# gattia/pyfocusr

Measured on AMD Instinct MI355X. Metric: lowest-k eigenpairs/sec + KNN-correspondence wall-clock, 250k-vertex mesh pair k=5, higher is better.
Workload: dtype f64

## Files before the change

### include/pyfocusr_hip.h

```cpp
#ifndef PYFOCUSR_HIP_H
#define PYFOCUSR_HIP_H

#include <stddef.h>
#include <stdint.h>

#ifdef __cplusplus
extern "C" {
#endif

#define PF_VERSION 1

#define PF_OK 0
#define PF_E_ARG (-1)
#define PF_E_HIP (-2)
#define PF_E_DEGENERATE (-3)
#define PF_E_STATE (-4)
#define PF_E_PERSIST_TIMEOUT (-5)

#define PF_OP_RW 0
#define PF_OP_SYM 1

typedef struct pf_ctx pf_ctx;
typedef struct pf_graph pf_graph;
typedef struct pf_mesh pf_mesh;
// ... 67 lines not shown
int pf_persist_enable(int on);
int pf_persist_two_step(int level);
int pf_persist_pair_halves(int on);
int pf_persist_clock(pf_ctx* ctx, double* kernel_ms, int64_t* launches, int reset);
typedef struct pf_persist_info {
    int32_t enabled;
    int32_t two_step;
    int32_t owner;
    int32_t timeouts;
    int64_t launches;
    int64_t launches_two_step;
    int32_t suspended_for;
    int32_t rearms;
    int32_t owner_switches;
    int32_t hold_ticks;
} pf_persist_info;
int pf_persist_state(pf_ctx* ctx , pf_persist_info* out);
int pf_persist_test_hook(int n_launches);
int pf_cheb(pf_graph* g, int32_t op, int32_t src, int32_t dst, int32_t degree, double c, double e, double rho);
int pf_cheb2(pf_graph* ga, int32_t op_a, int32_t src_a, int32_t dst_a, int32_t degree_a, double c_a, double e_a, double rho_a,
             pf_graph* gb, int32_t op_b, int32_t src_b, int32_t dst_b, int32_t degree_b, double c_b, double e_b, double rho_b);
int pf_dots(pf_graph* g, int32_t w, int32_t first, int32_t count, double* out);
int pf_orth(pf_graph* g, int32_t w, int32_t first, int32_t count, double* h, double* nrm);
int pf_orth_begin(pf_graph* g, int32_t w, int32_t first, int32_t count, int32_t normalize);
int pf_orth_end(pf_graph* g, double* h, double* nrm);
int pf_orth_begin2(pf_graph* ga, int32_t w_a, int32_t first_a, int32_t count_a, int32_t normalize_a, pf_graph* gb, int32_t w_b,
                   int32_t first_b, int32_t count_b, int32_t normalize_b);
int pf_orth_cheb2(pf_graph* ga, pf_graph* gb, const int32_t* orth, const int32_t* cheb_i, const double* cheb_d);
int pf_orth_redone(pf_graph* g);
int pf_orth_strict(pf_graph* g, int32_t on);
int pf_orth_device_passes(pf_graph* g, int32_t on);
int pf_orth_split(pf_graph* g, int32_t first2, int32_t split);
int pf_orth_one_launch(int32_t on);
int pf_scale(pf_graph* g, int32_t slot, double alpha);
int pf_combine(pf_graph* g, int32_t src_first, int32_t m, const double* Y, int32_t k, int32_t dst_first);
int pf_resnorm(pf_graph* g, int32_t ax, int32_t x, double lam, double* out);
int pf_gram(pf_graph* g, int32_t first_a, int32_t count_a, int32_t first_b, int32_t count_b, double* out);
int pf_resnorms(pf_graph* g, int32_t ax_first, int32_t x_first, const double* lam, int32_t count, double* out);
int pf_finalize_vectors(pf_graph* g, int32_t first, int32_t count, int32_t from_sym, int32_t minmax,
                        double* out);
int pf_finalize_vectors_begin(pf_graph* g, int32_t first, int32_t count, int32_t from_sym, int32_t minmax, double* out);
int pf_finalize_vectors_end(pf_graph* g);
int pf_final_remap_begin(pf_graph* g, const int32_t* col, const double* sign, int32_t count, double* out);
int pf_host_alloc(size_t bytes, void** out);
int pf_host_free(void* p);
int pf_host_detach(void* p);
int pf_final_rows(pf_graph* g, const int64_t* rows, int64_t n_rows, double* out);
int pf_point_rows(pf_graph* g, const int64_t* rows, int64_t n_rows, double* out);
int pf_spmv_host(pf_graph* g, int32_t op, const double* x, double* y);
int pf_mean_filter(pf_graph* g, const double* values, int32_t ncols, int32_t iterations, double* out);

int pf_knn1(pf_ctx* ctx, const double* ref, int64_t n_ref, const double* qry, int64_t n_qry, int32_t d,
            int64_t* idx_out, double* d2_out);
int pf_knn_mode(pf_ctx* ctx, int32_t mode);
int pf_knn_tree_stats(pf_ctx* ctx, int32_t enable_counting, int64_t* leaves_scanned, int64_t* supers_opened);
int pf_knn_count(pf_ctx* ctx, int32_t enable_counting, int64_t* pairs);
int pf_knn_wave_stats(pf_ctx* ctx, double* sum_us, double* max_us, int64_t* waves, int64_t* max_candidates, double* detail);
int pf_knn(pf_ctx* ctx, const double* ref, int64_t n_ref, const double* qry, int64_t n_qry, int32_t d, int32_t k,
           int64_t* idx_out, double* d2_out);
int pf_knn_topk(pf_ctx* ctx, const double* ref, int64_t n_ref, const double* qry, int64_t n_qry, int32_t d, int32_t k,
                int64_t* idx_out, double* d2_out);
int pf_knn1_graphs(pf_graph* ref_g, pf_graph* qry_g, int32_t d, const int32_t* col_ref, const double* scale_ref,
                   const int32_t* col_qry, const double* scale_qry, int64_t* idx_out, double* d2_out);
int pf_knn1_blocks(pf_ctx* ctx, const double* ref_block, int64_t n_ref, int32_t ref_stride, const double* qry_block,
                   int64_t n_qry, int32_t qry_stride, int32_t d, const int32_t* col_ref, const double* scale_ref,
                   const int32_t* col_qry, const double* scale_qry, int64_t* idx_out, double* d2_out);
// ... 132 lines not shown
```

### pyfocusr_amd/_hip.py

```python
import atexit
import ctypes as C
import os
import threading
import weakref

import numpy as np

_HERE = os.path.dirname(os.path.abspath(__file__))
LIB_PATH = os.environ.get("PYFOCUSR_HIP_LIB", os.path.join(_HERE, "csrc", "libpyfocusr_hip.so"))

PF_OP_RW = 0
PF_OP_SYM = 1

_f64p = C.POINTER(C.c_double)
_i32p = C.POINTER(C.c_int32)
_i64p = C.POINTER(C.c_int64)


class HipUnavailable(RuntimeError):
    pass


class PfError(RuntimeError):
    def __init__(self, code, msg):
# ... 51 lines not shown
    "pf_graph_build_cotan": (C.c_int, [C.c_void_p, C.c_int32, C.POINTER(C.c_void_p)]),
    "pf_graph_cotan_info": (C.c_int, [C.c_void_p, C.POINTER(C.c_double), C.POINTER(C.c_double)]),
    "pf_graph_cotan_download": (C.c_int, [C.c_void_p, _f64p, _f64p, _f64p]),
    "pf_cotan_apply": (C.c_int, [C.c_void_p, _f64p, C.c_int32, _f64p]),
    "pf_graph_free": (None, [C.c_void_p]),
    "pf_graph_get_info": (C.c_int, [C.c_void_p, C.POINTER(GraphInfo)]),
    "pf_graph_download": (C.c_int, [C.c_void_p, _i32p, _i32p, _f64p, _f64p, _f64p, _f64p, _i32p]),
    "pf_ws_ensure": (C.c_int, [C.c_void_p, C.c_int32]),
    "pf_ws_upload": (C.c_int, [C.c_void_p, C.c_int32, _f64p]),
    "pf_ws_download": (C.c_int, [C.c_void_p, C.c_int32, C.c_int32, _f64p]),
    "pf_ws_copy": (C.c_int, [C.c_void_p, C.c_int32, C.c_int32, C.c_int32]),
    "pf_start_vector": (C.c_int, [C.c_void_p, C.c_int32, C.c_uint64]),
    "pf_mask_isolated": (C.c_int, [C.c_void_p, C.c_int32]),
    "pf_lock_null_vectors": (C.c_int, [C.c_void_p, C.c_int32, _i32p]),
    "pf_spmv": (C.c_int, [C.c_void_p, C.c_int32, C.c_int32, C.c_int32]),
    "pf_spmv_multi": (C.c_int, [C.c_void_p, C.c_int32, C.c_int32, C.c_int32, C.c_int32]),
    "pf_knn_mode": (C.c_int, [C.c_void_p, C.c_int32]),
    "pf_knn_tree_stats": (C.c_int, [C.c_void_p, C.c_int32, C.POINTER(C.c_int64), C.POINTER(C.c_int64)]),
    "pf_persist_enable": (C.c_int, [C.c_int]),
    "pf_persist_two_step": (C.c_int, [C.c_int]),
    "pf_persist_pair_halves": (C.c_int, [C.c_int]),
    "pf_persist_clock": (C.c_int, [C.c_void_p, C.POINTER(C.c_double), C.POINTER(C.c_int64), C.c_int]),
    "pf_persist_state": (C.c_int, [C.c_void_p, C.c_void_p]),
    "pf_persist_test_hook": (C.c_int, [C.c_int]),
    "pf_cheb": (C.c_int, [C.c_void_p, C.c_int32, C.c_int32, C.c_int32, C.c_int32, C.c_double, C.c_double, C.c_double]),
    "pf_cheb2": (C.c_int, [C.c_void_p, C.c_int32, C.c_int32, C.c_int32, C.c_int32, C.c_double, C.c_double, C.c_double,
                           C.c_void_p, C.c_int32, C.c_int32, C.c_int32, C.c_int32, C.c_double, C.c_double, C.c_double]),
    "pf_dots": (C.c_int, [C.c_void_p, C.c_int32, C.c_int32, C.c_int32, _f64p]),
    "pf_orth": (C.c_int, [C.c_void_p, C.c_int32, C.c_int32, C.c_int32, _f64p, _f64p]),
    "pf_orth_begin": (C.c_int, [C.c_void_p, C.c_int32, C.c_int32, C.c_int32, C.c_int32]),
    "pf_orth_end": (C.c_int, [C.c_void_p, _f64p, _f64p]),
    "pf_orth_split": (C.c_int, [C.c_void_p, C.c_int32, C.c_int32]),
    "pf_orth_one_launch": (C.c_int, [C.c_int32]),
    "pf_orth_begin2": (C.c_int, [C.c_void_p, C.c_int32, C.c_int32, C.c_int32, C.c_int32, C.c_void_p, C.c_int32, C.c_int32, C.c_int32,
                                 C.c_int32]),
    "pf_orth_cheb2": (C.c_int, [C.c_void_p, C.c_void_p, _i32p, _i32p, _f64p]),
    "pf_eigsort_costs": (C.c_int, [C.c_void_p, C.c_void_p, _i64p, C.c_int64, _i64p, C.c_int64, C.c_int32, _i32p, _f64p, _i32p, _f64p, _f64p,
                                   _i64p]),
    "pf_orth_redone": (C.c_int, [C.c_void_p]),
    "pf_orth_strict": (C.c_int, [C.c_void_p, C.c_int32]),
    "pf_scale": (C.c_int, [C.c_void_p, C.c_int32, C.c_double]),
    "pf_combine": (C.c_int, [C.c_void_p, C.c_int32, C.c_int32, _f64p, C.c_int32, C.c_int32]),
    "pf_resnorm": (C.c_int, [C.c_void_p, C.c_int32, C.c_int32, C.c_double, _f64p]),
    "pf_gram": (C.c_int, [C.c_void_p, C.c_int32, C.c_int32, C.c_int32, C.c_int32, _f64p]),
    "pf_resnorms": (C.c_int, [C.c_void_p, C.c_int32, C.c_int32, _f64p, C.c_int32, _f64p]),
    "pf_finalize_vectors": (C.c_int, [C.c_void_p, C.c_int32, C.c_int32, C.c_int32, C.c_int32, _f64p]),
    "pf_finalize_vectors_begin": (C.c_int, [C.c_void_p, C.c_int32, C.c_int32, C.c_int32, C.c_int32, _f64p]),
    "pf_finalize_vectors_end": (C.c_int, [C.c_void_p]),
    "pf_final_remap_begin": (C.c_int, [C.c_void_p, _i32p, _f64p, C.c_int32, _f64p]),
    "pf_host_alloc": (C.c_int, [C.c_size_t, C.POINTER(C.c_void_p)]),
    "pf_host_free": (C.c_int, [C.c_void_p]),
    "pf_final_rows": (C.c_int, [C.c_void_p, _i64p, C.c_int64, _f64p]),
    "pf_point_rows": (C.c_int, [C.c_void_p, _i64p, C.c_int64, _f64p]),
    "pf_spmv_host": (C.c_int, [C.c_void_p, C.c_int32, _f64p, _f64p]),
    "pf_mean_filter": (C.c_int, [C.c_void_p, _f64p, C.c_int32, C.c_int32, _f64p]),
    "pf_knn1": (C.c_int, [C.c_void_p, _f64p, C.c_int64, _f64p, C.c_int64, C.c_int32, _i64p, _f64p]),
    "pf_knn": (C.c_int, [C.c_void_p, _f64p, C.c_int64, _f64p, C.c_int64, C.c_int32, C.c_int32, _i64p, _f64p]),
    "pf_knn_topk": (C.c_int, [C.c_void_p, _f64p, C.c_int64, _f64p, C.c_int64, C.c_int32, C.c_int32, _i64p, _f64p]),
    "pf_knn1_graphs": (C.c_int, [C.c_void_p, C.c_void_p, C.c_int32, _i32p, _f64p, _i32p, _f64p, _i64p, _f64p]),
    "pf_knn1_blocks": (C.c_int, [C.c_void_p, C.c_void_p, C.c_int64, C.c_int32, C.c_void_p, C.c_int64, C.c_int32, C.c_int32,
                                 _i32p, _f64p, _i32p, _f64p, _i64p, _f64p]),
    "pf_final_device": (C.c_int, [C.c_void_p, C.POINTER(C.c_void_p), _i64p, _i32p]),
    "pf_knn_upload": (C.c_int, [C.c_void_p, _f64p, C.c_int64, _f64p, C.c_int64, C.c_int32]),
    "pf_knn_run": (C.c_int, [C.c_void_p]),
    "pf_knn_download": (C.c_int, [C.c_void_p, _i64p, _f64p]),
    "pf_eigs_smallest": (C.c_int, [C.c_void_p, C.c_int32, C.c_int32, _f64p, _f64p, C.POINTER(C.c_int32), C.POINTER(EigsStats)]),
# ... 154 lines not shown
    for ptr in blocks:
        _lib.pf_host_free(C.c_void_p(ptr))


def pinned_empty(shape, dtype=np.float64):
    lib = load_library()
    dtype = np.dtype(dtype)
    count = int(np.prod(shape)) if len(shape) else 1
    nbytes = max(count * dtype.itemsize, 1)
    nbytes = (nbytes + 4095) & ~4095
    ptr = None
    with _pinned_lock:
        free = _pinned_free.get(nbytes)
        if free:
            ptr = free.pop()
            _pinned_cached[0] -= nbytes
    if ptr is None:
        p = C.c_void_p()
        _check(lib.pf_host_alloc(C.c_size_t(nbytes), C.byref(p)))
        ptr = int(p.value)
    buf = (C.c_char * nbytes).from_address(ptr)
    buf._pf_block = _PinnedBlock(ptr, nbytes)
    return np.frombuffer(buf, dtype=dtype, count=count).reshape(shape)


def persist_enable(on=True):
    _check(load_library().pf_persist_enable(int(bool(on))))


def orth_one_launch(on=True):
    _check(load_library().pf_orth_one_launch(int(bool(on))))


def persist_two_step(level=1):
    _check(load_library().pf_persist_two_step(int(level)))


def persist_pair_halves(on=True):
    _check(load_library().pf_persist_pair_halves(int(bool(on))))


def persist_clock(ctx, reset=False):
    ms, n = C.c_double(0.0), C.c_int64(0)
    _check(load_library().pf_persist_clock(ctx._h, C.byref(ms), C.byref(n), int(bool(reset))))
    return ms.value, n.value


class _PersistInfo(C.Structure):
    _fields_ = [("enabled", C.c_int32), ("two_step", C.c_int32), ("owner", C.c_int32), ("timeouts", C.c_int32),
                ("launches", C.c_int64), ("launches_two_step", C.c_int64), ("suspended_for", C.c_int32), ("rearms", C.c_int32),
                ("owner_switches", C.c_int32), ("hold_ticks", C.c_int32)]


def persist_state(ctx=None):
    info = _PersistInfo()
    _check(load_library().pf_persist_state(None if ctx is None else ctx._h, C.byref(info)))
    return {name: int(getattr(info, name)) for name, _ in _PersistInfo._fields_}


def persist_test_hook(n_launches=1):
    _check(load_library().pf_persist_test_hook(int(n_launches)))


def _check(code):
    if code != 0:
        raise PfError(code, load_library().pf_last_error().decode("utf-8", "replace"))
# ... 1035 lines not shown
```

### pyfocusr_amd/csrc/pf_eigsort.hip

```cpp
#include <float.h>
#include <string.h>

#include <vector>

#include "pf_internal.h"

extern "C" int pf_knn1_blocks(pf_ctx* c, const double* ref_block, int64_t n_ref, int32_t ref_stride, const double* qry_block, int64_t n_qry,
                              int32_t qry_stride, int32_t d, const int32_t* col_ref, const double* scale_ref, const int32_t* col_qry,
                              const double* scale_qry, int64_t* idx_out, double* d2_out);

namespace {

constexpr int ES_SORT_THREADS = 1024;
constexpr int ES_MAX_SAMPLES = 16384;
constexpr int ES_RED_THREADS = 256;

__global__ __launch_bounds__(PF_BLOCK) void k_es_gather(const double* __restrict__ fin, int32_t fc, const double* __restrict__ pts,
                                                        const int64_t* __restrict__ rows, int64_t m, int32_t k,
                                                        const int32_t* __restrict__ col, const double* __restrict__ sign,
                                                        double* __restrict__ vals, double* __restrict__ raw) {
    const int64_t e = (int64_t)blockIdx.x * PF_BLOCK + threadIdx.x;
    if (e >= m * (k + 3)) return;
    const int64_t c = e / m, r = e - c * m;
    if (c < k) vals[c * m + r] = fin[rows[r] * fc + col[c]] * sign[c];
// ... 3 lines not shown
__global__ __launch_bounds__(ES_RED_THREADS) void k_es_minmax(const double* __restrict__ raw, int64_t m, double* __restrict__ lohi) {
    __shared__ double slo[ES_RED_THREADS], shi[ES_RED_THREADS];
    const int c = blockIdx.x;
    double lo = INFINITY, hi = -INFINITY;
    for (int64_t r = threadIdx.x; r < m; r += ES_RED_THREADS) {
        const double v = raw[r * 3 + c];
        lo = v < lo ? v : lo;
        hi = v > hi ? v : hi;
    }
    slo[threadIdx.x] = lo;
    shi[threadIdx.x] = hi;
    __syncthreads();
    for (int s = ES_RED_THREADS / 2; s > 0; s >>= 1) {
        if (threadIdx.x < s) {
            slo[threadIdx.x] = slo[threadIdx.x + s] < slo[threadIdx.x] ? slo[threadIdx.x + s] : slo[threadIdx.x];
            shi[threadIdx.x] = shi[threadIdx.x + s] > shi[threadIdx.x] ? shi[threadIdx.x + s] : shi[threadIdx.x];
        }
        __syncthreads();
    }
    if (threadIdx.x == 0) {
        lohi[c] = slo[0];
        lohi[3 + c] = shi[0];
    }
}

__global__ __launch_bounds__(PF_BLOCK) void k_es_normalize(const double* __restrict__ raw, const double* __restrict__ lohi, int64_t m,
                                                           double* __restrict__ out) {
    const int64_t e = (int64_t)blockIdx.x * PF_BLOCK + threadIdx.x;
    if (e >= m * 3) return;
    const int c = (int)(e % 3);
    out[e] = (raw[e] - lohi[c]) / (lohi[3 + c] - lohi[c]);
}

__global__ __launch_bounds__(ES_SORT_THREADS) void k_es_sort_log(const double* __restrict__ vals_t, const double* __restrict__ vals_s,
                                                                 int64_t mt, int64_t ms, int32_t k, double* __restrict__ lt,
                                                                 double* __restrict__ ls, double* __restrict__ lsf) {
    extern __shared__ double buf[];
    const int b = blockIdx.x;
    const int64_t m = b < k ? mt : ms;
    int n_pow2 = 2;
    while (n_pow2 < m) n_pow2 <<= 1;
    const double* src = b < k ? vals_t + (int64_t)b * m : vals_s + (int64_t)(b - k) * m;
    for (int i = threadIdx.x; i < n_pow2; i += ES_SORT_THREADS) buf[i] = i < m ? src[i] : INFINITY;
    __syncthreads();
    for (int size = 2; size <= n_pow2; size <<= 1) {
        for (int stride = size >> 1; stride > 0; stride >>= 1) {
            for (int t = threadIdx.x; t < n_pow2 / 2; t += ES_SORT_THREADS) {
                const int pos = 2 * t - (t & (stride - 1));
                const double a = buf[pos], c = buf[pos + stride];
                const bool up = (pos & size) == 0;
                if ((a > c) == up) {
                    buf[pos] = c;
                    buf[pos + stride] = a;
                }
            }
            __syncthreads();
        }
    }
    const double eps = DBL_EPSILON;
    if (b < k) {
        for (int64_t i = threadIdx.x; i < m; i += ES_SORT_THREADS) lt[(int64_t)b * m + i] = log(buf[i] + 0.5 + eps);
    } else {
        const int64_t o = (int64_t)(b - k) * m;
        for (int64_t i = threadIdx.x; i < m; i += ES_SORT_THREADS) {
            ls[o + i] = log(buf[i] + 0.5 + eps);
            lsf[o + i] = log(-buf[m - 1 - i] + 0.5 + eps);
        }
    }
}

__device__ __forceinline__ double es_block_sum(double v, double* sh) {
    sh[threadIdx.x] = v;
    __syncthreads();
    for (int s = ES_RED_THREADS / 2; s > 0; s >>= 1) {
        if (threadIdx.x < s) sh[threadIdx.x] += sh[threadIdx.x + s];
        __syncthreads();
    }
    const double r = sh[0];
    __syncthreads();
    return r;
}

__global__ __launch_bounds__(ES_RED_THREADS) void k_es_w1(const double* __restrict__ lt, const double* __restrict__ ls,
                                                          const double* __restrict__ lsf, int64_t mt, int64_t ms, int32_t k,
                                                          double* __restrict__ out) {
    __shared__ double sh[ES_RED_THREADS];
    const int i = blockIdx.x / k, j = blockIdx.x - i * k;
    const double unit = 1.0 / ((double)mt * (double)ms);
    double acc = 0.0, accf = 0.0;
    for (int64_t a = threadIdx.x; a < mt; a += ES_RED_THREADS) {
        const double t = lt[(int64_t)i * mt + a];
        const int64_t lo = a * ms, hi = lo + ms;
        for (int64_t b = lo / mt; b < ms && b * mt < hi; ++b) {
            const int64_t from = b * mt > lo ? b * mt : lo, to = (b + 1) * mt < hi ? (b + 1) * mt : hi;
            const double len = (double)(to - from) * unit;
            acc += len * fabs(t - ls[(int64_t)j * ms + b]);
            accf += len * fabs(t - lsf[(int64_t)j * ms + b]);
        }
    }
    acc = es_block_sum(acc, sh);
    accf = es_block_sum(accf, sh);
// ... 14 lines not shown
        const double t = vals_t[(int64_t)i * m + r], s = (nn >= 0 && nn < ms) ? vals_s[(int64_t)j * ms + nn] : NAN;
        const double d0 = s - t, d1 = -s - t;
        a += d0 * d0;
        f += d1 * d1;
    }
    a = es_block_sum(a, sh);
    f = es_block_sum(f, sh);
    if (threadIdx.x == 0) {
        out[2 * k * k + i * k + j] = sqrt(a) / (double)m;
        out[3 * k * k + i * k + j] = sqrt(f) / (double)m;
    }
}

}

extern "C" int pf_eigsort_costs(pf_graph* gt, pf_graph* gs, const int64_t* rows_t, int64_t mt, const int64_t* rows_s, int64_t ms, int32_t k,
                                const int32_t* col_t, const double* sign_t, const int32_t* col_s, const double* sign_s, double* out,
                                int64_t* idx_out) {
    PF_CHECK(gt && gs && rows_t && rows_s && col_t && sign_t && col_s && sign_s && out && idx_out, PF_E_ARG,
             "pf_eigsort_costs: NULL argument");
    PF_CHECK(gt->ctx == gs->ctx, PF_E_ARG, "pf_eigsort_costs: the two graphs must share one ctx");
    PF_CHECK(mt >= 1 && mt <= ES_MAX_SAMPLES && ms >= 1 && ms <= ES_MAX_SAMPLES && k >= 1 && k <= 16, PF_E_ARG,
             "pf_eigsort_costs: %lld / %lld samples (1..%d), k = %d (1..16)", (long long)mt, (long long)ms, ES_MAX_SAMPLES, k);
    PF_CHECK(gt->final_vecs && gs->final_vecs, PF_E_STATE, "pf_eigsort_costs: no pf_finalize_vectors result is resident");
    PF_CHECK(gt->pts && gs->pts, PF_E_STATE, "pf_eigsort_costs: the graphs were not built from meshes");
    for (int32_t c = 0; c < k; ++c)
        PF_CHECK(col_t[c] >= 0 && col_t[c] < gt->final_count && col_s[c] >= 0 && col_s[c] < gs->final_count, PF_E_ARG,
                 "pf_eigsort_costs: column out of range");
    for (int64_t r = 0; r < mt; ++r) PF_CHECK(rows_t[r] >= 0 && rows_t[r] < gt->n, PF_E_ARG, "pf_eigsort_costs: sample row out of range");
    for (int64_t r = 0; r < ms; ++r) PF_CHECK(rows_s[r] >= 0 && rows_s[r] < gs->n, PF_E_ARG, "pf_eigsort_costs: sample row out of range");
    pf_ctx* c = gt->ctx;
    PF_HIP(hipSetDevice(c->device));
    hipStream_t st = c->stream;
    int32_t n_pow2 = 2;
    while (n_pow2 < (mt > ms ? mt : ms)) n_pow2 <<= 1;
    const size_t sort_lds = sizeof(double) * (size_t)n_pow2;
    if (sort_lds > 64 * 1024)
        PF_HIP(hipFuncSetAttribute(reinterpret_cast<const void*>(k_es_sort_log), hipFuncAttributeMaxDynamicSharedMemorySize,
                                   (int)(sizeof(double) * ES_MAX_SAMPLES)));

    const size_t head = sizeof(int64_t) * (size_t)(mt + ms);
    const size_t small = ((sizeof(int32_t) * 2 * k + 7) & ~(size_t)7) + sizeof(double) * 2 * k;
    std::vector<unsigned char> host(head + small);
    memcpy(host.data(), rows_t, sizeof(int64_t) * (size_t)mt);
    memcpy(host.data() + sizeof(int64_t) * (size_t)mt, rows_s, sizeof(int64_t) * (size_t)ms);
    int32_t* hcol = reinterpret_cast<int32_t*>(host.data() + head);
    double* hsign = reinterpret_cast<double*>(host.data() + head + ((sizeof(int32_t) * 2 * k + 7) & ~(size_t)7));
    for (int32_t i = 0; i < k; ++i) {
        hcol[i] = col_t[i];
        hcol[k + i] = col_s[i];
        hsign[i] = sign_t[i];
        hsign[k + i] = sign_s[i];
    }
    const size_t kt = (size_t)k * (size_t)mt, ks = (size_t)k * (size_t)ms;
    const size_t doubles = 2 * kt + 3 * ks + 6 * (size_t)(mt + ms) + 12 + 4 * (size_t)k * k;
    unsigned char* d = nullptr;
    const size_t up_bytes = (host.size() + 7) & ~(size_t)7, out_bytes = sizeof(double) * 4 * (size_t)k * k;
    unsigned char* pin = nullptr;
    PF_TRY(pf_pinned_scratch(c, up_bytes + out_bytes, reinterpret_cast<void**>(&pin)));
    memcpy(pin, host.data(), host.size());
    PF_HIP(pf_malloc(st, (void**)&d, up_bytes + sizeof(double) * doubles));
    int rc = PF_OK;
    do {
        auto fail = [&](hipError_t e) {
            if (e == hipSuccess) return false;
            pf_set_error("pf_eigsort_costs: %s", hipGetErrorString(e));
            rc = PF_E_HIP;
            return true;
        };
        if ((rc = pf_copy_by_kernel(st, pin, d, up_bytes)) != PF_OK) break;
        const int64_t* d_rows_t = reinterpret_cast<const int64_t*>(d);
        const int64_t* d_rows_s = d_rows_t + mt;
        const int32_t* d_col = reinterpret_cast<const int32_t*>(d + head);
        const double* d_sign = reinterpret_cast<const double*>(d + head + ((sizeof(int32_t) * 2 * k + 7) & ~(size_t)7));
        double* base = reinterpret_cast<double*>(d + up_bytes);
        double* vals_t = base;
        double* vals_s = vals_t + kt;
        double* raw_t = vals_s + ks;
        double* raw_s = raw_t + 3 * mt;
        double* norm_t = raw_s + 3 * ms;
        double* norm_s = norm_t + 3 * mt;
        double* lohi = norm_s + 3 * ms;
        double* lt = lohi + 12;
        double* ls = lt + kt;
        double* lsf = ls + ks;
        double* d_out = lsf + ks;
        k_es_gather<<<pf_blocks(mt * (k + 3)), PF_BLOCK, 0, st>>>(gt->final_vecs, gt->final_count, gt->pts, d_rows_t, mt, k, d_col, d_sign,
                                                                  vals_t, raw_t);
        k_es_gather<<<pf_blocks(ms * (k + 3)), PF_BLOCK, 0, st>>>(gs->final_vecs, gs->final_count, gs->pts, d_rows_s, ms, k, d_col + k,
                                                                  d_sign + k, vals_s, raw_s);
        k_es_minmax<<<3, ES_RED_THREADS, 0, st>>>(raw_t, mt, lohi);
        k_es_minmax<<<3, ES_RED_THREADS, 0, st>>>(raw_s, ms, lohi + 6);
        k_es_normalize<<<pf_blocks(3 * mt), PF_BLOCK, 0, st>>>(raw_t, lohi, mt, norm_t);
        k_es_normalize<<<pf_blocks(3 * ms), PF_BLOCK, 0, st>>>(raw_s, lohi + 6, ms, norm_s);
        k_es_sort_log<<<(unsigned)(2 * k), ES_SORT_THREADS, sort_lds, st>>>(vals_t, vals_s, mt, ms, k, lt, ls, lsf);
        k_es_w1<<<(unsigned)(k * k), ES_RED_THREADS, 0, st>>>(lt, ls, lsf, mt, ms, k, d_out);
        if (fail(hipGetLastError())) break;
        const int32_t cols3[3] = {0, 1, 2};
        const double ones3[3] = {1.0, 1.0, 1.0};
        rc = pf_knn1_blocks(c, norm_s, ms, 3, norm_t, mt, 3, 3, cols3, ones3, cols3, ones3, idx_out, nullptr);
        if (rc != PF_OK) break;
        k_es_spatial<<<(unsigned)(k * k), ES_RED_THREADS, 0, st>>>(vals_t, vals_s, c->knn_idx, mt, ms, k, d_out);
        if (fail(hipGetLastError())) break;
        if ((rc = pf_copy_by_kernel(st, d_out, pin + up_bytes, out_bytes)) != PF_OK) break;
        if (fail(hipStreamSynchronize(st))) break;
        memcpy(out, pin + up_bytes, out_bytes);
    } while (0);
    if (rc != PF_OK) (void)hipStreamSynchronize(st);
    pf_free(st, d);
    return rc;
}
```

### pyfocusr_amd/csrc/pf_operator.hip

```cpp
#include <math.h>
#include <stdlib.h>
#include <string.h>

#include <algorithm>
#include <atomic>
#include <map>
#include <mutex>
#include <vector>

#include "pf_internal.h"

namespace {

#ifndef PF_OP_BLOCK
#define PF_OP_BLOCK 256
#endif
struct OpArgs {
    const int64_t* slice_ptr;
    const int32_t* scol;
    const double* sval;
    const double* diag;
    const double* x;
    const double* prev;
    double* out;
// ... 520 lines not shown
}

__global__ __launch_bounds__(PF_BLOCK) void k_permute_in(const double* __restrict__ src_old, const int32_t* __restrict__ perm,
                                                         int64_t n_pad, double* __restrict__ dst_new) {
    const int64_t r = (int64_t)blockIdx.x * PF_BLOCK + threadIdx.x;
    if (r >= n_pad) return;
    const int32_t i = perm[r];
    dst_new[r] = i >= 0 ? src_old[i] : 0.0;
}

__global__ __launch_bounds__(PF_BLOCK) void k_permute_out(const double* __restrict__ ws, int64_t n_pad, int32_t first,
                                                          int32_t count, const int32_t* __restrict__ iperm, int64_t n,
                                                          double* __restrict__ dst_old ) {
    const int64_t i = (int64_t)blockIdx.x * PF_BLOCK + threadIdx.x;
    if (i >= n) return;
    const int64_t r = iperm[i];
    for (int c = 0; c < count; ++c) dst_old[(int64_t)c * n + i] = ws[(int64_t)(first + c) * n_pad + r];
}

__global__ __launch_bounds__(PF_BLOCK) void k_null_vector(double* __restrict__ x, const int32_t* __restrict__ label,
                                                          const int32_t* __restrict__ rowptr,
                                                          const double* __restrict__ deg, const int32_t* __restrict__ perm,
                                                          int64_t n_pad, int32_t root, int32_t sym,
                                                          const double* __restrict__ weight) {
    const int64_t r = (int64_t)blockIdx.x * PF_BLOCK + threadIdx.x;
    if (r >= n_pad) return;
    const int32_t i = perm[r];
    double v = 0.0;
    if (i >= 0 && label[i] == root && rowptr[i + 1] > rowptr[i]) v = weight ? weight[i] : (sym ? sqrt(deg[i] + 1e-8) : 1.0);
    x[r] = v;
}

constexpr int COMBINE_COLS = 8;
__global__ __launch_bounds__(PF_BLOCK) void k_combine(double* __restrict__ ws, int64_t n_pad, int32_t src_first, int32_t m,
                                                      const double* __restrict__ Y, int32_t k, int32_t c0, int32_t ncols,
                                                      int32_t dst_first, int32_t src_first2, int32_t dst_first2) {
    const int64_t i = (int64_t)blockIdx.x * PF_BLOCK + threadIdx.x;
    if (i >= n_pad) return;
    if (blockIdx.y) src_first = src_first2, dst_first = dst_first2;
    double acc[COMBINE_COLS];
#pragma unroll
    for (int c = 0; c < COMBINE_COLS; ++c) acc[c] = 0.0;
    for (int b = 0; b < m; ++b) {
        const double v = ws[(int64_t)(src_first + b) * n_pad + i];
        const double* yr = Y + (int64_t)b * k + c0;
#pragma unroll
        for (int c = 0; c < COMBINE_COLS; ++c)
            if (c < ncols) acc[c] += v * yr[c];
    }
#pragma unroll
    for (int c = 0; c < COMBINE_COLS; ++c)
        if (c < ncols) ws[(int64_t)(dst_first + c0 + c) * n_pad + i] = acc[c];
}

__global__ __launch_bounds__(PF_BLOCK) void k_resnorm_partial(const double* __restrict__ ax, const double* __restrict__ x,
                                                              double lam, int64_t n_pad, int64_t n_chunks,
                                                              double* __restrict__ partial) {
    __shared__ double red[PF_BLOCK / PF_WAVE];
    const int64_t lo = (int64_t)blockIdx.x * PF_DOT_CHUNK;
    const int64_t hi = lo + PF_DOT_CHUNK < n_pad ? lo + PF_DOT_CHUNK : n_pad;
    double s = 0.0;
    for (int64_t i = lo + threadIdx.x; i < hi; i += PF_BLOCK) {
        const double r = ax[i] - lam * x[i];
        s += r * r;
    }
#pragma unroll
    for (int off = PF_WAVE / 2; off > 0; off >>= 1) s += __shfl_down(s, off, PF_WAVE);
    if ((threadIdx.x & (PF_WAVE - 1)) == 0) red[threadIdx.x / PF_WAVE] = s;
    __syncthreads();
    if (threadIdx.x == 0) partial[blockIdx.x] = (red[0] + red[1]) + (red[2] + red[3]);
}

__global__ __launch_bounds__(PF_BLOCK) void k_gram_partial(const double* __restrict__ ws, int64_t n_pad, int32_t first_a, int32_t first_b,
                                                           int32_t count_b, int64_t n_chunks, double* __restrict__ partial) {
    __shared__ double red[PF_BLOCK / PF_WAVE];
    const int p = blockIdx.y;
    const int i = p / count_b, j = p - i * count_b;
    const double* v = ws + (int64_t)(first_b + j) * n_pad;
    const double* w = ws + (int64_t)(first_a + i) * n_pad;
    const int64_t lo = (int64_t)blockIdx.x * PF_DOT_CHUNK;
    const int64_t hi = lo + PF_DOT_CHUNK < n_pad ? lo + PF_DOT_CHUNK : n_pad;
    double s = 0.0;
    for (int64_t r = lo + 2 * threadIdx.x; r < hi; r += 2 * PF_BLOCK) {
        const double2 a = *reinterpret_cast<const double2*>(v + r);
        const double2 c = *reinterpret_cast<const double2*>(w + r);
// ... 419 lines not shown
int dots_device(pf_graph* g, int32_t w, int32_t first, int32_t count, double* d_out, double* d_acc, int accumulate) {
    hipStream_t st = g->ctx->stream;
    PF_TRY(pf_reduce_ensure(g, count));
    dim3 grid((unsigned)g->n_chunks, (unsigned)count);
    k_dot_partial<<<grid, PF_BLOCK, 0, st>>>(g->ws, g->n_pad, first, w, g->n_chunks, g->partials);
    PF_HIP(hipGetLastError());
    k_dot_finish<<<(unsigned)count, PF_WAVE, 0, st>>>(g->partials, g->n_chunks, d_out, d_acc, accumulate);
    PF_HIP(hipGetLastError());
    return PF_OK;
}

}

int pf_reduce_ensure(pf_graph* g, int32_t count) {
    if (count > g->partial_cap) {
        pf_free(g->ctx->stream, g->partials);
        g->partials = nullptr;
        const int32_t cap = std::max(count, 64);
        PF_HIP(pf_malloc(g->ctx->stream, (void**)&g->partials, sizeof(VecStats) * (size_t)cap * (size_t)(g->n_chunks + 1)));
        g->partial_cap = cap;
    }
    if (count > g->coef_cap) {
        pf_free(g->ctx->stream, g->coef);
        g->coef = nullptr;
        const int32_t cap = std::max(count, 64);
        PF_HIP(pf_malloc(g->ctx->stream, (void**)&g->coef, sizeof(double) * 8 * (size_t)cap));
        g->coef_cap = cap;
    }
    return PF_OK;
}

extern "C" {

int pf_ws_ensure(pf_graph* g, int32_t n_slots) {
    PF_CHECK(g != nullptr && n_slots > 0, PF_E_ARG, "pf_ws_ensure: bad argument");
    if (n_slots <= g->n_slots) return PF_OK;
    PF_HIP(hipSetDevice(g->ctx->device));
    hipStream_t st = g->ctx->stream;
    double* nw = nullptr;
    const size_t bytes = sizeof(double) * (size_t)(n_slots + PF_WS_TMPS) * (size_t)g->n_pad;
    PF_HIP(pf_malloc(st, (void**)&nw, bytes));
    PF_HIP(hipMemsetAsync(nw, 0, bytes, st));
    if (g->ws && g->n_slots > 0)
        PF_HIP(hipMemcpyAsync(nw, g->ws, sizeof(double) * (size_t)g->n_slots * g->n_pad, hipMemcpyDeviceToDevice, st));
    pf_free(st, g->ws);
    g->ws = nw;
    g->n_slots = n_slots;
    return PF_OK;
}

int pf_ws_upload(pf_graph* g, int32_t slot, const double* x) {
    PF_TRY(check_slots(g, slot, 1, "pf_ws_upload"));
    PF_CHECK(x != nullptr, PF_E_ARG, "pf_ws_upload: x is NULL");
    hipStream_t st = g->ctx->stream;
    PF_TRY(stage_ensure(g, g->n));
    PF_HIP(hipMemcpyAsync(g->stage, x, sizeof(double) * g->n, hipMemcpyHostToDevice, st));
    k_permute_in<<<pf_blocks(g->n_pad), PF_BLOCK, 0, st>>>(g->stage, g->perm, g->n_pad, pf_slot(g, slot));
    PF_HIP(hipGetLastError());
    PF_HIP(hipStreamSynchronize(st));
    return PF_OK;
}

int pf_ws_download(pf_graph* g, int32_t first, int32_t count, double* out) {
    PF_TRY(check_slots(g, first, count, "pf_ws_download"));
    PF_CHECK(out != nullptr, PF_E_ARG, "pf_ws_download: out is NULL");
    if (count == 0) return PF_OK;
    hipStream_t st = g->ctx->stream;
    PF_TRY(stage_ensure(g, (int64_t)count * g->n));
    k_permute_out<<<pf_blocks(g->n), PF_BLOCK, 0, st>>>(g->ws, g->n_pad, first, count, g->iperm, g->n, g->stage);
    PF_HIP(hipGetLastError());
    PF_HIP(hipMemcpyAsync(out, g->stage, sizeof(double) * (size_t)count * g->n, hipMemcpyDeviceToHost, st));
    PF_HIP(hipStreamSynchronize(st));
    return pf_persist_check(g->ctx);
}

// ... 512 lines not shown
    PF_TRY(pf_orth_begin(g, w, first, count, 0));
    return pf_orth_end(g, h, nrm);
}

int pf_scale(pf_graph* g, int32_t slot, double alpha) {
    PF_TRY(check_slots(g, slot, 1, "pf_scale"));
    k_scale<<<pf_blocks(g->n_pad), PF_BLOCK, 0, g->ctx->stream>>>(pf_slot(g, slot), g->n_pad, alpha);
    PF_HIP(hipGetLastError());
    return PF_OK;
}

int pf_combine(pf_graph* g, int32_t src_first, int32_t m, const double* Y, int32_t k, int32_t dst_first) {
    return pf_combine2(g, src_first, m, Y, k, dst_first, -1, -1);
}

}

int pf_combine2(pf_graph* g, int32_t src_first, int32_t m, const double* Y, int32_t k, int32_t dst_first, int32_t src_first2,
                int32_t dst_first2) {
    PF_TRY(check_slots(g, src_first, m, "pf_combine"));
    PF_TRY(check_slots(g, dst_first, k, "pf_combine"));
    PF_CHECK(Y != nullptr && m > 0 && k > 0, PF_E_ARG, "pf_combine: bad argument");
    PF_CHECK(src_first + m <= dst_first || dst_first + k <= src_first, PF_E_ARG, "pf_combine: overlapping ranges");
    const bool two = src_first2 >= 0;
    if (two) {
        PF_TRY(check_slots(g, src_first2, m, "pf_combine"));
        PF_TRY(check_slots(g, dst_first2, k, "pf_combine"));
        PF_CHECK((src_first2 + m <= dst_first2 || dst_first2 + k <= src_first2) && (dst_first + k <= dst_first2 || dst_first2 + k <= dst_first) &&
                     (src_first + m <= dst_first2 || dst_first2 + k <= src_first) && (src_first2 + m <= dst_first || dst_first + k <= src_first2),
                 PF_E_ARG, "pf_combine: overlapping ranges");
    }
    pf_ctx* ctx = g->ctx;
    hipStream_t st = ctx->stream;
    double* dY = nullptr;
    PF_HIP(pf_malloc(st, (void**)&dY, sizeof(double) * (size_t)m * k));
    const size_t bytes = sizeof(double) * (size_t)m * k;
    const void* src = Y;
    bool staged = false;
    if (bytes <= PF_STAGE_BYTES) {
        if (!ctx->stage_ring) {
            if (hipHostMalloc(&ctx->stage_ring, (size_t)PF_STAGE_SLOTS * PF_STAGE_BYTES, hipHostMallocDefault) != hipSuccess) {
                (void)hipGetLastError();
                ctx->stage_ring = nullptr;
            } else {
                for (int i = 0; i < PF_STAGE_SLOTS; ++i) ctx->stage_ev[i] = nullptr;
            }
        }
        if (ctx->stage_ring) {
            const int slot = ctx->stage_next;
            ctx->stage_next = (slot + 1) % PF_STAGE_SLOTS;
            bool ok = true;
            if (!ctx->stage_ev[slot]) ok = hipEventCreateWithFlags(&ctx->stage_ev[slot], hipEventDisableTiming) == hipSuccess;
            else ok = hipEventSynchronize(ctx->stage_ev[slot]) == hipSuccess;
            if (ok) {
                void* dst = static_cast<unsigned char*>(ctx->stage_ring) + (size_t)slot * PF_STAGE_BYTES;
                memcpy(dst, Y, bytes);
                src = dst;
                staged = true;
                hipError_t es = hipMemcpyAsync(dY, src, bytes, hipMemcpyHostToDevice, st);
                if (es == hipSuccess) es = hipEventRecord(ctx->stage_ev[slot], st);
                if (es != hipSuccess) {
                    pf_free(st, dY);
                    PF_HIP(es);
                }
            } else {
                (void)hipGetLastError();
// ... 662 lines not shown
```

Baseline: 998.6.

## Register bitonic sort, kernel-argument combine coefficients, drop workspace zero-fill

Rewrites the eigenvalue sort-log kernel as a register-resident bitonic sort with E elements per thread. Within a wavefront it exchanges through shuffles and uses LDS only for strides that cross waves, replacing the full-LDS network that synchronised at every stage. Small combine coefficient matrices (up to 256 entries) are passed by value as a kernel argument, which avoids a device malloc and host-to-device copy per combine call. The workspace memset on growth is removed unless a new poison debug flag is set, so newly grown workspace slots are left uninitialised and any code that relied on zeros could now read garbage.

```diff
diff --git a/include/pyfocusr_hip.h b/include/pyfocusr_hip.h
--- a/include/pyfocusr_hip.h
+++ b/include/pyfocusr_hip.h
@@ -123,6 +123,7 @@
 int pf_orth_device_passes(pf_graph* g, int32_t on);
 int pf_orth_split(pf_graph* g, int32_t first2, int32_t split);
 int pf_orth_one_launch(int32_t on);
+int pf_ws_poison(int32_t on);
 int pf_scale(pf_graph* g, int32_t slot, double alpha);
 int pf_combine(pf_graph* g, int32_t src_first, int32_t m, const double* Y, int32_t k, int32_t dst_first);
 int pf_resnorm(pf_graph* g, int32_t ax, int32_t x, double lam, double* out);
diff --git a/pyfocusr_amd/_hip.py b/pyfocusr_amd/_hip.py
--- a/pyfocusr_amd/_hip.py
+++ b/pyfocusr_amd/_hip.py
@@ -107,6 +107,7 @@
     "pf_orth_end": (C.c_int, [C.c_void_p, _f64p, _f64p]),
     "pf_orth_split": (C.c_int, [C.c_void_p, C.c_int32, C.c_int32]),
     "pf_orth_one_launch": (C.c_int, [C.c_int32]),
+    "pf_ws_poison": (C.c_int, [C.c_int32]),
     "pf_orth_begin2": (C.c_int, [C.c_void_p, C.c_int32, C.c_int32, C.c_int32, C.c_int32, C.c_void_p, C.c_int32, C.c_int32, C.c_int32,
                                  C.c_int32]),
     "pf_orth_cheb2": (C.c_int, [C.c_void_p, C.c_void_p, _i32p, _i32p, _f64p]),
@@ -327,6 +328,10 @@
     _check(load_library().pf_orth_one_launch(int(bool(on))))
 
 
+def ws_poison(on=True):
+    _check(load_library().pf_ws_poison(int(bool(on))))
+
+
 def persist_two_step(level=1):
     _check(load_library().pf_persist_two_step(int(level)))
 
diff --git a/pyfocusr_amd/csrc/pf_eigsort.hip b/pyfocusr_amd/csrc/pf_eigsort.hip
--- a/pyfocusr_amd/csrc/pf_eigsort.hip
+++ b/pyfocusr_amd/csrc/pf_eigsort.hip
@@ -59,41 +59,80 @@
     out[e] = (raw[e] - lohi[c]) / (lohi[3 + c] - lohi[c]);
 }
 
+__device__ __forceinline__ double es_cx(double mine, double other, bool low, bool up) {
+    const double a = low ? mine : other, c = low ? other : mine;
+    return ((a > c) == up) ? other : mine;
+}
+
+template <int E>
 __global__ __launch_bounds__(ES_SORT_THREADS) void k_es_sort_log(const double* __restrict__ vals_t, const double* __restrict__ vals_s,
                                                                  int64_t mt, int64_t ms, int32_t k, double* __restrict__ lt,
                                                                  double* __restrict__ ls, double* __restrict__ lsf) {
     extern __shared__ double buf[];
-    const int b = blockIdx.x;
+    constexpr int N = E * ES_SORT_THREADS;
+    const int b = blockIdx.x, t = threadIdx.x;
     const int64_t m = b < k ? mt : ms;
-    int n_pow2 = 2;
-    while (n_pow2 < m) n_pow2 <<= 1;
     const double* src = b < k ? vals_t + (int64_t)b * m : vals_s + (int64_t)(b - k) * m;
-    for (int i = threadIdx.x; i < n_pow2; i += ES_SORT_THREADS) buf[i] = i < m ? src[i] : INFINITY;
-    __syncthreads();
-    for (int size = 2; size <= n_pow2; size <<= 1) {
-        for (int stride = size >> 1; stride > 0; stride >>= 1) {
-            for (int t = threadIdx.x; t < n_pow2 / 2; t += ES_SORT_THREADS) {
-                const int pos = 2 * t - (t & (stride - 1));
-                const double a = buf[pos], c = buf[pos + stride];
-                const bool up = (pos & size) == 0;
-                if ((a > c) == up) {
-                    buf[pos] = c;
-                    buf[pos + stride] = a;
+    double v[E];
+#pragma unroll
+    for (int j = 0; j < E; ++j) v[j] = t * E + j < m ? src[t * E + j] : INFINITY;
+    for (int size = 2; size <= N; size <<= 1) {
+        int stride = size >> 1;
+        for (; stride >= PF_WAVE * E; stride >>= 1) {
+            const int dt = stride / E;
+            const bool low = (t & dt) == 0;
+#pragma unroll
+            for (int j = 0; j < E; ++j) buf[j * ES_SORT_THREADS + t] = v[j];
+            __syncthreads();
+#pragma unroll
+            for (int j = 0; j < E; ++j) v[j] = es_cx(v[j], buf[j * ES_SORT_THREADS + (t ^ dt)], low, ((t * E + j) & size) == 0);
+            __syncthreads();
+        }
+        for (; stride >= E; stride >>= 1) {
+            const int dt = stride / E;
+            const bool low = (t & dt) == 0;
+#pragma unroll
+            for (int j = 0; j < E; ++j) v[j] = es_cx(v[j], __shfl_xor(v[j], dt, PF_WAVE), low, ((t * E + j) & size) == 0);
+        }
+#pragma unroll
+        for (int s = E / 2; s > 0; s >>= 1) {
+            if (s > stride) continue;
+#pragma unroll
+            for (int j = 0; j < E; ++j) {
+                if (j & s) continue;
+                const double a = v[j], c = v[j | s];
+                if ((a > c) == (((t * E + j) & size) == 0)) {
+                    v[j] = c;
+                    v[j | s] = a;
                 }
             }
-            __syncthreads();
         }
     }
     const double eps = DBL_EPSILON;
-    if (b < k) {
-        for (int64_t i = threadIdx.x; i < m; i += ES_SORT_THREADS) lt[(int64_t)b * m + i] = log(buf[i] + 0.5 + eps);
-    } else {
-        const int64_t o = (int64_t)(b - k) * m;
-        for (int64_t i = threadIdx.x; i < m; i += ES_SORT_THREADS) {
-            ls[o + i] = log(buf[i] + 0.5 + eps);
-            lsf[o + i] = log(-buf[m - 1 - i] + 0.5 + eps);
-        }
-    }
+    const int64_t o = b < k ? (int64_t)b * m : (int64_t)(b - k) * m;
+#pragma unroll
+    for (int j = 0; j < E; ++j) {
+        const int64_t i = t * E + j;
+        if (i >= m) continue;
+        if (b < k) {
+            lt[o + i] = log(v[j] + 0.5 + eps);
+        } else {
+            ls[o + i] = log(v[j] + 0.5 + eps);
+            lsf[o + m - 1 - i] = log(-v[j] + 0.5 + eps);
+        }
+    }
+}
+
+template <int E>
+hipError_t es_sort_log(hipStream_t st, const double* vals_t, const double* vals_s, int64_t mt, int64_t ms, int32_t k, double* lt, double* ls,
+                       double* lsf) {
+    constexpr size_t lds = sizeof(double) * (size_t)E * ES_SORT_THREADS;
+    if (lds > 64 * 1024) {
+        const hipError_t e = hipFuncSetAttribute(reinterpret_cast<const void*>(k_es_sort_log<E>), hipFuncAttributeMaxDynamicSharedMemorySize, (int)lds);
+        if (e != hipSuccess) return e;
+    }
+    k_es_sort_log<E><<<(unsigned)(2 * k), ES_SORT_THREADS, lds, st>>>(vals_t, vals_s, mt, ms, k, lt, ls, lsf);
+    return hipSuccess;
 }
 
 __device__ __forceinline__ double es_block_sum(double v, double* sh) {
@@ -174,12 +213,8 @@
     pf_ctx* c = gt->ctx;
     PF_HIP(hipSetDevice(c->device));
     hipStream_t st = c->stream;
-    int32_t n_pow2 = 2;
-    while (n_pow2 < (mt > ms ? mt : ms)) n_pow2 <<= 1;
-    const size_t sort_lds = sizeof(double) * (size_t)n_pow2;
-    if (sort_lds > 64 * 1024)
-        PF_HIP(hipFuncSetAttribute(reinterpret_cast<const void*>(k_es_sort_log), hipFuncAttributeMaxDynamicSharedMemorySize,
-                                   (int)(sizeof(double) * ES_MAX_SAMPLES)));
+    int32_t sort_elems = 1;
+    while ((int64_t)sort_elems * ES_SORT_THREADS < (mt > ms ? mt : ms)) sort_elems <<= 1;
 
     const size_t head = sizeof(int64_t) * (size_t)(mt + ms);
     const size_t small = ((sizeof(int32_t) * 2 * k + 7) & ~(size_t)7) + sizeof(double) * 2 * k;
@@ -235,7 +270,15 @@
         k_es_minmax<<<3, ES_RED_THREADS, 0, st>>>(raw_s, ms, lohi + 6);
         k_es_normalize<<<pf_blocks(3 * mt), PF_BLOCK, 0, st>>>(raw_t, lohi, mt, norm_t);
         k_es_normalize<<<pf_blocks(3 * ms), PF_BLOCK, 0, st>>>(raw_s, lohi + 6, ms, norm_s);
-        k_es_sort_log<<<(unsigned)(2 * k), ES_SORT_THREADS, sort_lds, st>>>(vals_t, vals_s, mt, ms, k, lt, ls, lsf);
+        hipError_t es = hipSuccess;
+        switch (sort_elems) {
+            case 1: es = es_sort_log<1>(st, vals_t, vals_s, mt, ms, k, lt, ls, lsf); break;
+            case 2: es = es_sort_log<2>(st, vals_t, vals_s, mt, ms, k, lt, ls, lsf); break;
+            case 4: es = es_sort_log<4>(st, vals_t, vals_s, mt, ms, k, lt, ls, lsf); break;
+            case 8: es = es_sort_log<8>(st, vals_t, vals_s, mt, ms, k, lt, ls, lsf); break;
+            default: es = es_sort_log<16>(st, vals_t, vals_s, mt, ms, k, lt, ls, lsf); break;
+        }
+        if (fail(es)) break;
         k_es_w1<<<(unsigned)(k * k), ES_RED_THREADS, 0, st>>>(lt, ls, lsf, mt, ms, k, d_out);
         if (fail(hipGetLastError())) break;
         const int32_t cols3[3] = {0, 1, 2};
diff --git a/pyfocusr_amd/csrc/pf_operator.hip b/pyfocusr_amd/csrc/pf_operator.hip
--- a/pyfocusr_amd/csrc/pf_operator.hip
+++ b/pyfocusr_amd/csrc/pf_operator.hip
@@ -576,9 +576,13 @@
 }
 
 constexpr int COMBINE_COLS = 8;
-__global__ __launch_bounds__(PF_BLOCK) void k_combine(double* __restrict__ ws, int64_t n_pad, int32_t src_first, int32_t m,
-                                                      const double* __restrict__ Y, int32_t k, int32_t c0, int32_t ncols,
-                                                      int32_t dst_first, int32_t src_first2, int32_t dst_first2) {
+constexpr int COMBINE_ARG_MAX = 256;
+struct CombineY {
+    double y[COMBINE_ARG_MAX];
+};
+__device__ __forceinline__ void combine_rows(double* __restrict__ ws, int64_t n_pad, int32_t src_first, int32_t m,
+                                             const double* __restrict__ Y, int32_t k, int32_t c0, int32_t ncols, int32_t dst_first,
+                                             int32_t src_first2, int32_t dst_first2) {
     const int64_t i = (int64_t)blockIdx.x * PF_BLOCK + threadIdx.x;
     if (i >= n_pad) return;
     if (blockIdx.y) src_first = src_first2, dst_first = dst_first2;
@@ -595,6 +599,16 @@
 #pragma unroll
     for (int c = 0; c < COMBINE_COLS; ++c)
         if (c < ncols) ws[(int64_t)(dst_first + c0 + c) * n_pad + i] = acc[c];
+}
+__global__ __launch_bounds__(PF_BLOCK) void k_combine(double* __restrict__ ws, int64_t n_pad, int32_t src_first, int32_t m,
+                                                      const double* __restrict__ Y, int32_t k, int32_t c0, int32_t ncols,
+                                                      int32_t dst_first, int32_t src_first2, int32_t dst_first2) {
+    combine_rows(ws, n_pad, src_first, m, Y, k, c0, ncols, dst_first, src_first2, dst_first2);
+}
+__global__ __launch_bounds__(PF_BLOCK) void k_combine_arg(double* __restrict__ ws, int64_t n_pad, int32_t src_first, int32_t m,
+                                                          const CombineY Y, int32_t k, int32_t c0, int32_t ncols, int32_t dst_first,
+                                                          int32_t src_first2, int32_t dst_first2) {
+    combine_rows(ws, n_pad, src_first, m, Y.y, k, c0, ncols, dst_first, src_first2, dst_first2);
 }
 
 __global__ __launch_bounds__(PF_BLOCK) void k_resnorm_partial(const double* __restrict__ ax, const double* __restrict__ x,
@@ -1080,6 +1094,13 @@
 
 extern "C" {
 
+static std::atomic<int> g_ws_poison{0};
+
+int pf_ws_poison(int32_t on) {
+    g_ws_poison.store(on ? 1 : 0);
+    return PF_OK;
+}
+
 int pf_ws_ensure(pf_graph* g, int32_t n_slots) {
     PF_CHECK(g != nullptr && n_slots > 0, PF_E_ARG, "pf_ws_ensure: bad argument");
     if (n_slots <= g->n_slots) return PF_OK;
@@ -1088,7 +1109,7 @@
     double* nw = nullptr;
     const size_t bytes = sizeof(double) * (size_t)(n_slots + PF_WS_TMPS) * (size_t)g->n_pad;
     PF_HIP(pf_malloc(st, (void**)&nw, bytes));
-    PF_HIP(hipMemsetAsync(nw, 0, bytes, st));
+    if (g_ws_poison.load()) PF_HIP(hipMemsetAsync(nw, 0xFF, bytes, st));
     if (g->ws && g->n_slots > 0)
         PF_HIP(hipMemcpyAsync(nw, g->ws, sizeof(double) * (size_t)g->n_slots * g->n_pad, hipMemcpyDeviceToDevice, st));
     pf_free(st, g->ws);
@@ -1667,6 +1688,17 @@
     }
     pf_ctx* ctx = g->ctx;
     hipStream_t st = ctx->stream;
+    if ((int64_t)m * k <= COMBINE_ARG_MAX) {
+        CombineY ya;
+        memcpy(ya.y, Y, sizeof(double) * (size_t)m * k);
+        for (int32_t c0 = 0; c0 < k; c0 += COMBINE_COLS) {
+            const int32_t nc = std::min(COMBINE_COLS, k - c0);
+            k_combine_arg<<<dim3(pf_blocks(g->n_pad), two ? 2u : 1u), PF_BLOCK, 0, st>>>(g->ws, g->n_pad, src_first, m, ya, k, c0, nc, dst_first,
+                                                                                      src_first2, dst_first2);
+            PF_HIP(hipGetLastError());
+        }
+        return PF_OK;
+    }
     double* dY = nullptr;
     PF_HIP(pf_malloc(st, (void**)&dY, sizeof(double) * (size_t)m * k));
     const size_t bytes = sizeof(double) * (size_t)m * k;
```

Measured after the change: 1002, median of 3. About the same (+0.4%).
